# matsengrp/linearham

Measured on AMD Instinct MI355X. Metric: phylo-HMM log-likelihood evals/sec (100-leaf x 400-site family), higher is better.
Workload: dtype f64

## Files before the change

### linearham_amd/csrc/lh_prune.hip

```cpp
#include <cstdlib>

#include <cstdio>

#include "lh_device.h"

namespace lh {

namespace {

thread_local char g_prune_form[64] = "";
thread_local char g_prune_error[256] = "";

#define LH_SLOT_COPY(dst, src)                       \
  _Pragma("unroll") for (int s_ = 0; s_ < S; ++s_) { \
    dst[s_][0] = src[s_][0];                         \
    dst[s_][1] = src[s_][1];                         \
    dst[s_][2] = src[s_][2];                         \
    dst[s_][3] = src[s_][3];                         \
  }
#define LH_PUSH_IF(d)                                   \
  if constexpr (kDepth > d) {                           \
    if (push_mask & (1u << d)) { LH_SLOT_COPY(st##d, a) } \
  }
#define LH_POP_CASE(d)          \
  case d:                       \
    if constexpr (kDepth > d) { \
      LH_SLOT_COPY(y, st##d)    \
    }                           \
    break;
#define LH_POP_SLOT(d) \
  _Pragma("unroll") for (int s_ = 0; s_ < S; ++s_) matvec(pa, st##d[s_], z[s_]);
#define LH_DECL(d) double st##d[S][4];

typedef const double __attribute__((address_space(4))) * pmat_ptr;


__device__ __forceinline__ pmat_ptr pmat_after_barrier(const double* p) {
  const uint64_t bits = reinterpret_cast<uint64_t>(p);
  const uint32_t lo = (uint32_t)__builtin_amdgcn_readfirstlane((int)(uint32_t)bits);
  const uint32_t hi = (uint32_t)__builtin_amdgcn_readfirstlane((int)(uint32_t)(bits >> 32));
  uint64_t v = (uint64_t)lo | ((uint64_t)hi << 32);
  asm volatile("; lh: P-matrix scratch base %0 -- scalar loads of the walk depend on this statement" : "+s"(v) : : "memory");
  return (pmat_ptr)v;
}

__device__ __forceinline__ void matvec(pmat_ptr p, const double (&a)[4], double (&x)[4]) {
  x[0] = fma(p[3], a[3], fma(p[2], a[2], fma(p[1], a[1], p[0] * a[0])));
  x[1] = fma(p[7], a[3], fma(p[6], a[2], fma(p[5], a[1], p[4] * a[0])));
  x[2] = fma(p[11], a[3], fma(p[10], a[2], fma(p[9], a[1], p[8] * a[0])));
  x[3] = fma(p[15], a[3], fma(p[14], a[2], fma(p[13], a[1], p[12] * a[0])));
}

template <bool kN>
__device__ __forceinline__ void tip_column(const double* tiptab, int tip, int st, double (&c)[4], int ones_off) {
  const int off = tip * 16 + st * 4;
// ... 199 lines not shown
  const double2 q0 = q[0], q1 = q[1];
  c[0] = q0.x, c[1] = q0.y, c[2] = q1.x, c[3] = q1.y;
}

typedef int2 WalkOp;
enum : int { WOP_MATRIX = 8, WOP_PUSH_SHIFT = 4, WOP_POP_SHIFT = 9, WOP_HAS_B = 1 << 13, WOP_HAS_C = 1 << 14 };


template <bool kN>
__device__ __forceinline__ void tip_column_at(const char* tiptab_bytes, int entry_off, int st, double (&c)[4], int ones_off) {
  const int off = entry_off + st * 32;
  const double2* q = reinterpret_cast<const double2*>(tiptab_bytes + ((kN && st == 4) ? ones_off * 8 : off));
  const double2 q0 = q[0], q1 = q[1];
  c[0] = q0.x, c[1] = q0.y, c[2] = q1.x, c[3] = q1.y;
}

template <bool kN>
__device__ __forceinline__ void table_entry_at(const char* ctab_bytes, unsigned table_off, int sy, int sz, double (&c)[4]) {
  constexpr int SY = kN ? 5 : 4;
  const unsigned off = table_off + (unsigned)(sy * SY + sz) * 32u;
  const double2* q = reinterpret_cast<const double2*>(ctab_bytes + off);
  const double2 q0 = q[0], q1 = q[1];
  c[0] = q0.x, c[1] = q0.y, c[2] = q1.x, c[3] = q1.y;
}

template <int S>
__device__ __forceinline__ void close_naive_branch(const double (&a)[S][4], const int (&scal)[S], const double* naive_tab,
                                                   const double* __restrict__ p4, double (&lik)[S][5], int (&scl)[S]) {
#pragma unroll
  for (int s = 0; s < S; ++s) {
    const double w0 = p4[0] * a[s][0], w1 = p4[1] * a[s][1], w2 = p4[2] * a[s][2], w3 = p4[3] * a[s][3];
#pragma unroll
    for (int b = 0; b < 5; ++b) {
      double tv[4];
      if (b < 4) {
#pragma unroll
        for (int i = 0; i < 4; ++i) tv[i] = naive_tab[b * 4 + i];
      } else {
#pragma unroll
        for (int i = 0; i < 4; ++i) tv[i] = ((naive_tab[i] + naive_tab[4 + i]) + naive_tab[8 + i]) + naive_tab[12 + i];
      }
      lik[s][b] = fma(w3, tv[3], fma(w2, tv[2], fma(w1, tv[1], w0 * tv[0])));
    }
    scl[s] = scal[s];
  }
}

typedef __attribute__((address_space(5))) char* private_ptr;
typedef __attribute__((address_space(3))) const char* lds_ptr;

template <int kDepth, bool kN, int S>
__device__ __forceinline__ void prune_wave_asm(int block128, const uint64_t* __restrict__ planes, int n_blocks, int n_w,
                                               const WalkOp* __restrict__ wops, pmat_ptr pm, unsigned ctoff,
                                               const double* tiptab, const double* naive_tab, const double* ones,
                                               const double* __restrict__ p4, double (&lik)[S][5], int (&scl)[S]) {
  static_assert(S == 1 || S == 2, "one or two sites per lane");
  __attribute__((aligned(16))) double out_mem[4 * S + 2];
  __attribute__((aligned(16))) double deep_mem[(kDepth > 2 ? kDepth - 2 : 1) * 4 * S];
  constexpr int kMasks = kN ? 6 : 4;
  const int blk = min(block128, n_blocks - 1);
  const uint64_t* planes_w = planes + ((ptrdiff_t)blk - (ptrdiff_t)n_blocks) * kMasks;
  const unsigned pstride = (unsigned)n_blocks * (unsigned)(kMasks * 8);
  const unsigned tip_lds = (unsigned)(size_t)(lds_ptr)tiptab;
  if constexpr (kN && S == 2) {
    const unsigned ones_lds = (unsigned)(size_t)(lds_ptr)ones;
    asm volatile(
#include "lh_prune_walk_asm_s2n.inc"
        :
        : [nw] "s"(n_w), [wops] "s"(wops), [pm] "s"(pm), [ctoff] "s"(ctoff), [planes] "s"(planes_w), [pstride] "s"(pstride),
          [tip] "s"(tip_lds), [ones] "v"(ones_lds), [out] "v"((private_ptr)out_mem), [deep] "v"((private_ptr)deep_mem)
        : "memory", "vcc", "scc",
#include "lh_prune_walk_clobbers_s2.inc"
    );
  } else if constexpr (S == 2) {
    asm volatile(
#include "lh_prune_walk_asm_s2.inc"
        :
        : [nw] "s"(n_w), [wops] "s"(wops), [pm] "s"(pm), [ctoff] "s"(ctoff), [planes] "s"(planes_w), [pstride] "s"(pstride),
          [tip] "s"(tip_lds), [out] "v"((private_ptr)out_mem), [deep] "v"((private_ptr)deep_mem)
        : "memory", "vcc", "scc",
#include "lh_prune_walk_clobbers_s2.inc"
    );
  } else if constexpr (kN) {
    const unsigned ones_lds = (unsigned)(size_t)(lds_ptr)ones;
    asm volatile(
#include "lh_prune_walk_asm_s1n.inc"
        :
        : [nw] "s"(n_w), [wops] "s"(wops), [pm] "s"(pm), [ctoff] "s"(ctoff), [planes] "s"(planes_w), [pstride] "s"(pstride),
          [tip] "s"(tip_lds), [ones] "v"(ones_lds), [out] "v"((private_ptr)out_mem), [deep] "v"((private_ptr)deep_mem)
        : "memory", "vcc", "scc",
#include "lh_prune_walk_clobbers_s1.inc"
    );
  } else {
    asm volatile(
#include "lh_prune_walk_asm_s1.inc"
        :
        : [nw] "s"(n_w), [wops] "s"(wops), [pm] "s"(pm), [ctoff] "s"(ctoff), [planes] "s"(planes_w), [pstride] "s"(pstride),
          [tip] "s"(tip_lds), [out] "v"((private_ptr)out_mem), [deep] "v"((private_ptr)deep_mem)
        : "memory", "vcc", "scc",
#include "lh_prune_walk_clobbers_s1.inc"
    );
  }
  double a[S][4];
  int scal[S];
#pragma unroll
  for (int s = 0; s < S; ++s)
#pragma unroll
    for (int i = 0; i < 4; ++i) a[s][i] = out_mem[s * 4 + i];
  const unsigned* packed = reinterpret_cast<const unsigned*>(out_mem + 4 * S);
#pragma unroll
  for (int s = 0; s < S; ++s) scal[s] = (int)((packed[s / 2] >> (16 * (s & 1))) & 0xffffu);
  close_naive_branch<S>(a, scal, naive_tab, p4, lik, scl);
}

template <int kDepth, int S, bool kN>
__device__ __forceinline__ void prune_wave_ct(int site0, int site_end, const uint8_t* __restrict__ msa, int L, int n_w,
                                              const WalkOp* desc , pmat_ptr pm, const double* tiptab,
                                              const double* ctab, const double* naive_tab, int ones_off,
                                              const double* __restrict__ p4, double (&lik)[S][5], int (&scl)[S]) {
  constexpr unsigned kTabBytes = (kN ? 25 : 16) * 32;
  unsigned usite[S];
#pragma unroll
  for (int s = 0; s < S; ++s) {
    const int site = site0 + 64 * s;
    usite[s] = (unsigned)(site < site_end ? site : site_end - 1);
  }
  double a[S][4];
  int scal[S];
#pragma unroll
  for (int s = 0; s < S; ++s) {
    a[s][0] = a[s][1] = a[s][2] = a[s][3] = 1.0;
    scal[s] = 0;
  }
  double st0[S][4];
  double deep[kDepth > 1 ? kDepth - 1 : 1][S][4];
#pragma unroll
  for (int s = 0; s < S; ++s) st0[s][0] = st0[s][1] = st0[s][2] = st0[s][3] = 0.0;
  const char* tipb = reinterpret_cast<const char*>(tiptab);
  const char* ctabb = reinterpret_cast<const char*>(ctab);
  const uint8_t* msa_m = msa - L;
  const int last = n_w > 0 ? n_w - 1 : 0;
  WalkOp d0, d1, dv;
  {
    const WalkOp t0 = desc[0], t1 = desc[last < 1 ? last : 1];
    d0.x = __builtin_amdgcn_readfirstlane(t0.x), d0.y = __builtin_amdgcn_readfirstlane(t0.y);
    d1.x = __builtin_amdgcn_readfirstlane(t1.x), d1.y = __builtin_amdgcn_readfirstlane(t1.y);
    dv = desc[last < 2 ? last : 2];
  }
  int sa[S], sb[S], sc[S];
#pragma unroll
  for (int s = 0; s < S; ++s) sa[s] = sb[s] = sc[s] = 0;
  if (n_w > 0) {
#pragma unroll
    for (int s = 0; s < S; ++s) {
      sa[s] = msa_m[(unsigned)(((unsigned)d0.x >> 16) * L) + usite[s]];
      sb[s] = msa_m[(unsigned)((d0.y & 0xffff) * L) + usite[s]];
      sc[s] = msa_m[(unsigned)(((unsigned)d0.y >> 16) * L) + usite[s]];
    }
  }
  unsigned pm_off = 0, tab_off = 0;
  for (int k = 0; k < n_w; ++k) {
    const int kind = d0.x & 7;
    const int tip_a = (unsigned)d0.x >> 16, tip_b = d0.y & 0xffff, tip_c = (unsigned)d0.y >> 16;
    double x[S][4];
    if (d0.x & WOP_MATRIX) {
// ... 438 lines not shown
      atomicOr(err_flag, 1);
    } else {
      hdr[smp] = make_int4(c_wi, c_mi, c_ti, 0);
    }
  }
  if (any_bad) return;
  __syncthreads();
  for (int c = lane; c < c_ti; c += 64) ml[c_mi + c] = bl[tnode[c]];
}

__global__ void __launch_bounds__(64) schedule_stack_check_kernel(int T, int slots, int check_ranks,
                                                                  const int32_t* __restrict__ ops, int4* __restrict__ hdr,
                                                                  int32_t* err_flag) {
  const int smp = blockIdx.x, lane = threadIdx.x;
  const int n_ops = T - 2, nodes = 2 * T - 2;
  const int4* __restrict__ o = reinterpret_cast<const int4*>(ops) + (size_t)smp * n_ops;
  int carry = 0, depth0 = 0;
  bool bad = false;
  for (int k0 = 0; k0 < n_ops; k0 += 64) {
    const int k = k0 + lane;
    const bool in = k < n_ops;
    const int4 op = in ? o[k] : make_int4(OP_CHERRY, 1, 1, 0);
    const int kind = op.x & 15, rank = op.x >> OP_RANK_SHIFT;
    const bool push = (op.x & OP_PUSH_FLAG) != 0;
    bool ok = op.x >= 0 && (op.x & 0xe0) == 0 && kind <= OP_POP_ACC;
    if (kind == OP_CHERRY) ok = ok && op.y >= 1 && op.y < T && op.z >= 1 && op.z < T && push == (k != 0);
    if (kind == OP_TIP_ACC) ok = ok && !push && k > 0 && op.y >= 1 && op.y < T && op.z >= T && op.z < nodes;
    if (kind == OP_POP_ACC) ok = ok && !push && k > 0 && op.y >= T && op.y < nodes && op.z >= T && op.z < nodes;
    if (push || kind == OP_POP_ACC) ok = ok && op.w >= 0 && op.w < slots;
    const int m = !in || !ok ? 0 : kind == OP_TIP_ACC ? 1 : kind == OP_POP_ACC ? 2 : 0;
    const int dl = !in || !ok ? 0 : push ? 1 : kind == OP_POP_ACC ? -1 : 0;
    int incl = m, dincl = dl;
#pragma unroll
    for (int d = 1; d < 64; d <<= 1) {
      const int up = __shfl_up(incl, d), dup = __shfl_up(dincl, d);
      if (lane >= d) incl += up, dincl += dup;
    }
    const int depth = depth0 + dincl - dl;
    if (in && push && op.w != depth) ok = false;
    if (in && kind == OP_POP_ACC && op.w != depth - 1) ok = false;
    if (check_ranks && in && kind != OP_CHERRY && rank != carry + incl - m) ok = false;
    if (in && !ok) bad = true;
    carry += __shfl(incl, 63);
    depth0 += __shfl(dincl, 63);
  }
  if (carry != T - 3 || depth0 != 0) bad = true;
  const bool any_bad = __builtin_amdgcn_ballot_w64(bad) != 0;
  if (lane == 0) {
    hdr[smp] = make_int4(0, 0, 0, any_bad ? 1 : 0);
    if (any_bad) atomicOr(err_flag, 1);
  }
}

template <int kDepth, bool kN, bool kFused, bool kAsm = false>
__device__ __forceinline__ void prune_body_ct(int n2, int tile, int R, int wpr, const uint8_t* __restrict__ msa,
                                              const uint64_t* __restrict__ planes, int L,
                                              int T, const int2* __restrict__ wops, const double* __restrict__ wlen,
                                              const int4* __restrict__ tabs, int tabs_stride,
                                              const int4* __restrict__ hdr, const double* __restrict__ brlen,
                                              const double* __restrict__ rates, const double* __restrict__ eig,
                                              double* pmat_w, size_t rate_stride, const double* __restrict__ pi,
                                              double* __restrict__ site_lik, int32_t* __restrict__ site_scal) {
  extern __shared__ double2 smem2[];
  constexpr int SY = kN ? 5 : 4, E = SY * SY;
  const int tid = threadIdx.x;
  const int wave_all = __builtin_amdgcn_readfirstlane(tid >> 6);
  const int rate = kFused ? wave_all / wpr : (int)blockIdx.y;
  const int wave = kFused ? wave_all - rate * wpr : wave_all;
  const int nthr = kFused ? wpr * 64 : (int)blockDim.x;
  const int rtid = kFused ? tid - rate * nthr : tid;
  const int sample = blockIdx.z;
  const int n_ops = T - 2;
  const int4 h = hdr[sample];
  const int n_w = __builtin_amdgcn_readfirstlane(h.x);
  const int n_mat = __builtin_amdgcn_readfirstlane(h.y), n_tab = __builtin_amdgcn_readfirstlane(h.z);
  const bool malformed = h.w != 0;
  double* pw = pmat_w + ((size_t)sample * R + rate) * rate_stride;
  double* ctab = pw + (size_t)(T - 3 > 0 ? T - 3 : 0) * 16;
  constexpr int kS = 2;
  double* tiptab = reinterpret_cast<double*>(smem2) + (kFused ? (size_t)rate * T * 16 : 0);
  const double* naive_tab = tiptab;
  double* ones = reinterpret_cast<double*>(smem2) + (size_t)(kFused ? R : 1) * T * 16;
  const int ones_off = (int)(ones - tiptab);
  if (kN && tid < 4) ones[tid] = 1.0;
  const int4* __restrict__ tl = tabs + (size_t)sample * tabs_stride;
  WalkOp* desc = reinterpret_cast<WalkOp*>(reinterpret_cast<double*>(smem2) + (size_t)(kFused ? R : 1) * T * 16 + (kN ? 4 : 0));
  for (int i = tid; i < n_w; i += blockDim.x) desc[i] = wops[(size_t)sample * n_ops + i];

  const int n_q = min(n_tab, nthr >> 2);
  const bool pc_lane = (rtid & 3) == 0 && (rtid >> 2) < n_q;
  int4 tcell = make_int4(1, 1, 0, 0);
  if ((rtid >> 2) < n_q) tcell = tl[rtid >> 2];
  double pcq[16];
#pragma unroll
  for (int i = 0; i < 16; ++i) pcq[i] = 0.0;
  {
    const double* __restrict__ e = eig + (size_t)sample * 36;
    const double* __restrict__ bl = brlen + (size_t)sample * (2 * (size_t)T - 2);
    const double* __restrict__ wl = wlen + (size_t)sample * n_ops;
    const int n_rest = n_tab - n_q;
    const int n_list = n_mat + n_rest + T;
    const int round1 = nthr - n_q;
    auto item = [&](bool is_pc, int it, int rr, int quad) {
      double P[4][4];
      const bool in_list = !is_pc && it < n_list;
      const bool inner = in_list && it < n_mat + n_rest;
      const int slot = it < n_mat ? it : it + n_q;
      const int j = it - (n_mat + n_rest);
      double t = 0.0;
      if (is_pc) t = wl[n_mat + quad];
      else if (inner) t = wl[slot];
      else if (in_list) t = bl[j];
      compute_pmatrix(e, t * rates[(size_t)sample * R + rr], P);
      if (is_pc) {
#pragma unroll
        for (int i = 0; i < 4; ++i)
#pragma unroll
          for (int q = 0; q < 4; ++q) pcq[i * 4 + q] = P[i][q];
      } else if (inner) {
        double* o = pmat_w + ((size_t)sample * R + rr) * rate_stride + (size_t)slot * 16;
#pragma unroll
        for (int i = 0; i < 4; ++i)
#pragma unroll
          for (int q = 0; q < 4; ++q) o[i * 4 + q] = P[i][q];
      } else if (in_list) {
        double* o = reinterpret_cast<double*>(smem2) + (kFused ? (size_t)rr * T * 16 : 0) + j * 16;
#pragma unroll
        for (int i = 0; i < 4; ++i)
#pragma unroll
          for (int st = 0; st < 4; ++st) o[st * 4 + i] = P[i][st];
      }
    };
    const int rem = n_list - round1;
    if (rem > 0) {
      if constexpr (kFused) {
        const float inv_rem = 1.0f / (float)rem;
        for (int c = tid; c < R * rem; c += blockDim.x) {
          int rr = min((int)(((float)c + 0.5f) * inv_rem), R - 1);
          rr -= rr * rem > c ? 1 : 0;
          rr += (rr + 1) * rem <= c ? 1 : 0;
          item(false, round1 + c - rr * rem, rr, 0);
        }
      } else {
        for (int it = round1 + rtid; it < n_list; it += nthr) item(false, it, rate, 0);
      }
    }
    item(pc_lane, rtid - min(n_q, (rtid + 3) >> 2), rate, rtid >> 2);
  }
  if (n_tab > n_q) asm volatile("s_waitcnt vmcnt(0)" ::: "memory");
  asm volatile("s_waitcnt lgkmcnt(0)\n\ts_barrier" ::: "memory");
  auto build_rows = [&](const double (&pc)[16], int c, int sy, int ty, int tz) {
    double py[4];
    tip_column<kN>(tiptab, ty, sy, py, ones_off);
    double2* o = reinterpret_cast<double2*>(ctab) + ((size_t)c * E + (size_t)sy * SY) * 2;
#pragma unroll
    for (int sz = 0; sz < SY; ++sz) {
      double pz[4], pr[4], x[4];
      tip_column<kN>(tiptab, tz, sz, pz, ones_off);
#pragma unroll
      for (int i = 0; i < 4; ++i) pr[i] = py[i] * pz[i];
      matvec_v(pc, pr, x);
      o[2 * sz] = make_double2(x[0], x[1]);
      o[2 * sz + 1] = make_double2(x[2], x[3]);
    }
  };
  {
    double pc[16];
#pragma unroll
    for (int i = 0; i < 16; ++i) {
      const int lo = __builtin_amdgcn_mov_dpp(__double2loint(pcq[i]), 0, 0xf, 0xf, true);
      const int hi = __builtin_amdgcn_mov_dpp(__double2hiint(pcq[i]), 0, 0xf, 0xf, true);
      pc[i] = __hiloint2double(hi, lo);
    }
    if ((rtid >> 2) < n_q) {
      build_rows(pc, rtid >> 2, rtid & 3, tcell.x, tcell.y);
      if constexpr (kN) {
        const int sz = rtid & 3;
        double2* o = reinterpret_cast<double2*>(ctab) + ((size_t)(rtid >> 2) * E + 4 * SY) * 2;
        for (int k = sz; k < SY; k += 4) {
          double pz[4], pr[4], x[4];
          tip_column<kN>(tiptab, tcell.y, k, pz, ones_off);
#pragma unroll
          for (int i = 0; i < 4; ++i) pr[i] = 1.0 * pz[i];
          matvec_v(pc, pr, x);
          o[2 * k] = make_double2(x[0], x[1]);
          o[2 * k + 1] = make_double2(x[2], x[3]);
        }
      }
    }
  }
  for (int it = rtid; it < (n_tab - n_q) * SY; it += nthr) {
    const int c = n_q + it / SY, sy = it - (it / SY) * SY;
    const int4 t = tl[c];
    double pc[16];
    const double2* q = reinterpret_cast<const double2*>(pw + (size_t)(n_mat + c) * 16);
#pragma unroll
    for (int j = 0; j < 8; ++j) {
      const double2 v = q[j];
      pc[2 * j] = v.x;
      pc[2 * j + 1] = v.y;
    }
    build_rows(pc, c, sy, t.x, t.y);
  }
  asm volatile("s_waitcnt vmcnt(0)" ::: "memory");
  __threadfence_block();
  __syncthreads();

  const pmat_ptr pm = pmat_after_barrier(pw);
  const int lane = tid & 63;
  const int tile0 = blockIdx.x * tile;
  const int site_end = min(tile0 + tile, L);
  const double* __restrict__ p4 = pi + (size_t)sample * 4;
  double lik[kS][5];
  int scl[kS];
#pragma unroll
  for (int s = 0; s < kS; ++s) scl[s] = 0;
  int site0, n_own;
  const bool two_sites = wave < n2;
  if (two_sites) {
    site0 = tile0 + wave * (64 * kS) + lane;
    n_own = kS;
    if constexpr (kAsm)
      prune_wave_asm<kDepth, kN, kS>((tile0 + wave * (64 * kS)) >> 7, planes, (L + 127) >> 7, n_w, wops + (size_t)sample * n_ops, pm,
                                     (unsigned)((T - 3 > 0 ? T - 3 : 0) * 128), tiptab, naive_tab, ones, p4, lik, scl);
    else
      prune_wave_ct<kDepth, kS, kN>(site0, site_end, msa, L, n_w, desc, pm, tiptab, ctab, naive_tab, ones_off, p4, lik, scl);
  } else {
    site0 = tile0 + n2 * (64 * kS) + (wave - n2) * 64 + lane;
    n_own = 1;
    double lik1[1][5];
    int scl1[1];
    if constexpr (kAsm)
      prune_wave_asm<kDepth, kN, 1>((tile0 + n2 * (64 * kS)) >> 7, planes, (L + 127) >> 7, n_w,
                                    wops + (size_t)sample * n_ops, pm, (unsigned)((T - 3 > 0 ? T - 3 : 0) * 128), tiptab, naive_tab,
                                    ones, p4, lik1, scl1);
    else
      prune_wave_ct<kDepth, 1, kN>(site0, site_end, msa, L, n_w, desc, pm, tiptab, ctab, naive_tab, ones_off, p4, lik1, scl1);
#pragma unroll
    for (int b = 0; b < 5; ++b) lik[0][b] = lik1[0][b];
    scl[0] = scl1[0];
  }
  if (malformed) {
#pragma unroll
    for (int s = 0; s < kS; ++s)
#pragma unroll
      for (int b = 0; b < 5; ++b) lik[s][b] = __builtin_nan("");
  }

  if constexpr (!kFused) {
    double* lik_out = site_lik + (((size_t)sample * R + rate) * 5) * (size_t)L;
    int32_t* scal_out = site_scal + ((size_t)sample * R + rate) * (size_t)L;
#pragma unroll
    for (int s = 0; s < kS; ++s) {
      const int site = site0 + 64 * s;
      if (s < n_own && site < site_end) {
#pragma unroll
        for (int b = 0; b < 5; ++b) lik_out[(size_t)b * L + site] = lik[s][b];
        scal_out[site] = scl[s];
      }
    }
  } else {
    const int pad = n2 * (64 * kS) + (wpr - n2) * 64;
    __syncthreads();
    double* X = reinterpret_cast<double*>(smem2);
    int* SC = reinterpret_cast<int*>(X + (size_t)R * 5 * pad);
#pragma unroll
    for (int s = 0; s < kS; ++s) {
      const int idx = site0 + 64 * s - tile0;
      if (s < n_own && idx < pad) {
#pragma unroll
        for (int b = 0; b < 5; ++b) X[((size_t)rate * 5 + b) * pad + idx] = lik[s][b];
        SC[rate * pad + idx] = scl[s];
      }
    }
    __syncthreads();
    const int n_tile = site_end - tile0;
    const double w = 1.0 / R;
    double* lik_out = site_lik + ((size_t)sample * 5) * (size_t)L;
    int32_t* scal_out = site_scal + (size_t)sample * (size_t)L;
    for (int p = tid; p < n_tile; p += blockDim.x) {
      int smin = 0x7fffffff;
      for (int r = 0; r < R; ++r) smin = min(smin, SC[r * pad + p]);
      double acc[5] = {0.0, 0.0, 0.0, 0.0, 0.0};
      for (int r = 0; r < R; ++r) {
        const int d = SC[r * pad + p] - smin;
#pragma unroll
        for (int b = 0; b < 5; ++b) {
          double v = X[((size_t)r * 5 + b) * pad + p];
          for (int q = 0; q < d && v != 0.0; ++q) v *= kScaleThreshold;
          acc[b] += w * v;
        }
      }
#pragma unroll
      for (int b = 0; b < 5; ++b) lik_out[(size_t)b * L + tile0 + p] = acc[b];
      scal_out[tile0 + p] = smin;
    }
  }
}

#define LH_PRUNE_CT_PARAMS                                                                                          \
  int n2, int tile, int R, int wpr, const uint8_t *__restrict__ msa, const uint64_t *__restrict__ planes, int L,    \
      int T, const int2 *__restrict__ wops,                                                                         \
      const double *__restrict__ wlen, const int4 *__restrict__ tabs, int tabs_stride,                              \
      const int4 *__restrict__ hdr, const double *__restrict__ brlen, const double *__restrict__ rates,            \
      const double *__restrict__ eig, double *pmat_w, size_t rate_stride, const double *__restrict__ pi,           \
      double *__restrict__ site_lik, int32_t *__restrict__ site_scal
#define LH_PRUNE_CT_ARGS \
  n2, tile, R, wpr, msa, planes, L, T, wops, wlen, tabs, tabs_stride, hdr, brlen, rates, eig, pmat_w, rate_stride, pi, site_lik, \
      site_scal
#define LH_PRUNE_CT_KERNEL(NAME, WAVES)                                                              \
  template <int kDepth, bool kN, bool kFused, bool kAsm>                                             \
  __global__ void __launch_bounds__(1024) __attribute__((amdgpu_waves_per_eu(WAVES, WAVES))) NAME(   \
      LH_PRUNE_CT_PARAMS) {                                                                          \
    prune_body_ct<kDepth, kN, kFused, kAsm>(LH_PRUNE_CT_ARGS);                                       \
  }
LH_PRUNE_CT_KERNEL(prune_kernel_ct6, 6)
LH_PRUNE_CT_KERNEL(prune_kernel_ct5, 5)
LH_PRUNE_CT_KERNEL(prune_kernel_ct4, 4)
#undef LH_PRUNE_CT_KERNEL
#define LH_PRUNE_PARAMS                                                                                     \
  int n_samples, int n2, int tile, int R, int wpr, const uint8_t *__restrict__ msa, int L, int T, int n_ops, \
      const int32_t *__restrict__ ops, const int4 *__restrict__ hdr, int32_t *err_flag,                     \
      const double *__restrict__ brlen, const double *__restrict__ rates, const double *__restrict__ eig,  \
      double *pmat_w, size_t rate_stride, const double *__restrict__ pi,                                   \
      double *__restrict__ site_lik, int32_t *__restrict__ site_scal
#define LH_PRUNE_ARGS \
  n2, tile, R, wpr, msa, L, T, n_ops, ops, hdr, err_flag, brlen, rates, eig, pmat_w, rate_stride, pi, site_lik, site_scal
#define LH_PRUNE_SAMPLES(BODY) BODY((int)blockIdx.z, LH_PRUNE_ARGS);

#define LH_PRUNE_KERNEL(NAME, WAVES)                                                                 \
  template <int kDepth, bool kN>                                                                     \
  __global__ void __launch_bounds__(1024) __attribute__((amdgpu_waves_per_eu(WAVES, WAVES))) NAME(   \
      LH_PRUNE_PARAMS) {                                                                             \
    LH_PRUNE_SAMPLES((prune_body<kDepth, true, kN, true>))                                           \
  }
LH_PRUNE_KERNEL(prune_kernel_w6, 6)
LH_PRUNE_KERNEL(prune_kernel_w5, 5)
LH_PRUNE_KERNEL(prune_kernel_w4, 4)
#undef LH_PRUNE_KERNEL

template <int kDepth, bool kN>
__global__ void __launch_bounds__(512) __attribute__((amdgpu_waves_per_eu(5, 5))) prune_kernel_seg(LH_PRUNE_PARAMS) {
  LH_PRUNE_SAMPLES((prune_body<kDepth, true, kN, false, true>))
}
template <int kDepth, bool kN>
__global__ void __launch_bounds__(512) __attribute__((amdgpu_waves_per_eu(4, 4))) prune_kernel_seg4(LH_PRUNE_PARAMS) {
  LH_PRUNE_SAMPLES((prune_body<kDepth, true, kN, false, true>))
}

PruneWsSizes prune_ws_sizes(int T, bool mixed_n) {
  PruneWsSizes z;
  z.tabs_per_sample = (size_t)std::max((T - 1) / 2, 1);
  const size_t e = mixed_n ? 25 : 16;
  z.scratch_doubles_per_rate = std::max((size_t)std::max(T - 3, 0) * 16 + z.tabs_per_sample * e * 4, (size_t)std::max(T - 2, 1) * 32);
  return z;
}

int launch_prune(const DevFamily& fam, int n, int R, int T, int max_depth, const int32_t* ops,
                 const double* brlen, const double* rates, const double* eig, const PruneWs& ws, const double* pi,
                 double* site_lik, int32_t* site_scal, hipStream_t stream, bool allow_fused) {
  const int L = fam.n_prune;
  const PruneWsSizes sizes = prune_ws_sizes(T, fam.msa_mixed_n != 0);
  if (L == 0) {
    hipLaunchKernelGGL(schedule_stack_check_kernel, dim3(n), dim3(64), 0, stream, T, std::max(max_depth, 1), 0, ops, ws.hdr, ws.err_flag);
    return R;
  }
  double* pmat = ws.scratch;
  const size_t rate_stride = sizes.scratch_doubles_per_rate;
  const DebugOptions& dbg = debug_options();
  const int cap_env = dbg.k1_tile_cap;
  const int cap = cap_env >= 64 ? std::min(cap_env, 1024) : 1024;
  const int tiles = (L + cap - 1) / cap;
  const int tile = tiles == 1 ? L : (((L + tiles - 1) / tiles + 127) & ~127);
  int n2 = tile / 128, n1;
  {
    const int rem = tile - 128 * n2;
    if (rem > 64) {
      ++n2;
      n1 = 0;
    } else {
      n1 = rem > 0 ? 1 : 0;
    }
  }
  const int wpr = n2 + n1;
  const size_t tip_bytes = (size_t)T * 16 * sizeof(double);
  const size_t pad = (size_t)n2 * 128 + (size_t)n1 * 64;
  const size_t tail_bytes = (((size_t)std::max(T - 2, 1) * sizeof(int2)) + 31) & ~(size_t)15;
  const bool mixed = fam.msa_mixed_n != 0;
  const size_t ones_bytes = mixed ? 32 : 0;
  const size_t fused_lds = std::max((size_t)R * tip_bytes + ones_bytes + tail_bytes, (size_t)R * pad * (5 * sizeof(double) + sizeof(int)));
  const bool fused = allow_fused && !dbg.k1_no_fuse && !dbg.k1_segments &&
                     ((R * wpr <= 8 && fused_lds <= 53 * 1024) ||
                      (R * wpr > 8 && R * wpr <= 16 && fused_lds <= 80 * 1024));
  const bool big = !fused && ((160 * 1024 / tip_bytes) * wpr / 4 < 5 || dbg.k1_segments);
  const bool tables_hook = dbg.k1_tables || dbg.k1_no_tables;
  const bool use_asm = !dbg.k1_cxx_walk;
  const bool stack_fused = fused && max_depth <= 4 && dbg.k1_stack && !tables_hook;
  const bool seg = big && max_depth <= 4 && !tables_hook;
  const size_t seg_bytes = (size_t)(2 * kSegOps + 1) * 16 * sizeof(double) + ones_bytes;
  size_t lds = fused ? fused_lds : seg ? seg_bytes : tip_bytes + ones_bytes + tail_bytes;
  if (lds > 160 * 1024) {
    snprintf(g_prune_error, sizeof(g_prune_error),
             "K1: a tree of %d tips with stack depth %d needs %zu bytes of LDS in the cherry-table form (160 KB per CU)", T, max_depth, lds);
    return -1;
  }
  if (stack_fused || seg) {
    hipLaunchKernelGGL(schedule_stack_check_kernel, dim3(n), dim3(64), 0, stream, T, stack_fused && max_depth <= 3 ? 3 : 4,
                       stack_fused ? 1 : 0, ops, ws.hdr, ws.err_flag);
  } else {
    hipLaunchKernelGGL(schedule_rewrite_kernel, dim3(n), dim3(64), (sizes.tabs_per_sample + 16) * sizeof(int), stream, T, max_depth,
                       (int)sizes.tabs_per_sample, dbg.k1_no_tables ? 0 : 1, ops, brlen, ws.wops, ws.wlen, ws.tabs, ws.hdr, ws.err_flag);
  }
  const int wg_waves = fused ? R * wpr : wpr;
  dim3 grid(tiles, fused ? 1 : R, n), block(64 * wg_waves);
  const int n_ops = T - 2;
  hipError_t attr_rc = hipSuccess;
#define LH_LAUNCH_K(K, NAME)                                                                                     \
  {                                                                                                              \
    if (lds > 64 * 1024)                                                                                         \
      attr_rc = hipFuncSetAttribute(reinterpret_cast<const void*>(K), hipFuncAttributeMaxDynamicSharedMemorySize, (int)lds); \
    snprintf(g_prune_form, sizeof(g_prune_form), "%s", NAME);                                                    \
    if (attr_rc == hipSuccess)                                                                                   \
      hipLaunchKernelGGL(K, grid, block, lds, stream, n, n2, tile, R, wpr, fam.msa, L, T, n_ops, ops, ws.hdr, ws.err_flag, \
                         brlen, rates, eig, pmat, rate_stride, pi, site_lik, site_scal);                        \
  }
#define LH_LAUNCH_CT(K, NAME)                                                                                    \
  {                                                                                                              \
    if (lds > 64 * 1024)                                                                                         \
      attr_rc = hipFuncSetAttribute(reinterpret_cast<const void*>(K), hipFuncAttributeMaxDynamicSharedMemorySize, (int)lds); \
    snprintf(g_prune_form, sizeof(g_prune_form), "%s", NAME);                                                    \
    if (attr_rc == hipSuccess)                                                                                   \
      hipLaunchKernelGGL(K, grid, block, lds, stream, n2, tile, R, wpr, fam.msa, fam.msa_planes, L, T, ws.wops, ws.wlen, ws.tabs, \
                         (int)sizes.tabs_per_sample, ws.hdr, brlen, rates, eig, pmat, rate_stride, pi, site_lik, \
                         site_scal);                                                                             \
  }
  const int lds_waves = lds == 0 ? 8 : (int)((160 * 1024 / lds) * wg_waves / 4);
  if (stack_fused) {
#define LH_LAUNCH_STACK(D, N)                                                          \
  {                                                                                    \
    if (lds_waves >= 6 && D == 3)                                                      \
      LH_LAUNCH_K((prune_kernel_w6<D, N>), "w6<" #D "," #N ">")                        \
    else if (lds_waves >= 5)                                                           \
      LH_LAUNCH_K((prune_kernel_w5<D, N>), "w5<" #D "," #N ">")                        \
    else                                                                               \
      LH_LAUNCH_K((prune_kernel_w4<D, N>), "w4<" #D "," #N ">")                        \
  }
    if (max_depth <= 3 && !mixed)
      LH_LAUNCH_STACK(3, false)
    else if (max_depth <= 3)
      LH_LAUNCH_STACK(3, true)
    else if (!mixed)
      LH_LAUNCH_STACK(4, false)
    else
      LH_LAUNCH_STACK(4, true)
#undef LH_LAUNCH_STACK
  } else if (seg) {
    if (dbg.k1_seg_waves == 4) {
      if (mixed)
        LH_LAUNCH_K((prune_kernel_seg4<4, true>), "seg4<4,true>")
      else
        LH_LAUNCH_K((prune_kernel_seg4<4, false>), "seg4<4,false>")
    } else {
      if (mixed)
        LH_LAUNCH_K((prune_kernel_seg<4, true>), "seg5<4,true>")
      else
        LH_LAUNCH_K((prune_kernel_seg<4, false>), "seg5<4,false>")
    }
  } else {
#define LH_LAUNCH_BUDGET(D, N, F, A)                                                          \
  {                                                                                           \
    if (lds_waves >= 6)                                                                       \
      LH_LAUNCH_CT((prune_kernel_ct6<D, N, F, A>), "ct6<" #D "," #N "," #F "," #A ">")        \
    else if (lds_waves >= 5)                                                                  \
      LH_LAUNCH_CT((prune_kernel_ct5<D, N, F, A>), "ct5<" #D "," #N "," #F "," #A ">")        \
    else                                                                                      \
      LH_LAUNCH_CT((prune_kernel_ct4<D, N, F, A>), "ct4<" #D "," #N "," #F "," #A ">")        \
  }
#define LH_LAUNCH_FORM(D, N, A)        \
  {                                    \
    if (fused)                         \
      LH_LAUNCH_BUDGET(D, N, true, A)  \
    else                               \
      LH_LAUNCH_BUDGET(D, N, false, A) \
  }
#define LH_LAUNCH_SHALLOW(D)           \
  {                                    \
    if (mixed && use_asm)              \
      LH_LAUNCH_FORM(D, true, true)    \
// ... 30 lines not shown
```

Before: 8.107 million.

## Re-read kernel arguments from kernarg segment to cut SGPR/VGPR pressure in prune_body_ct

Packs the prune kernel's many parameters into a struct and has the body reload fields from the kernarg segment (through opaque asm barriers) per phase instead of keeping them live across the asm walk. The naive-branch closing is moved out of the asm wave routine so the walk's register footprint shrinks. It also replaces the integer divide for the fused rate index with a loop or rcp-based estimate and rolls the table-building loop for the non-quad path. The aim is lower register pressure and fewer live values across the barrier, traded for extra scalar loads and some added complexity and risk.

```diff
diff --git a/linearham_amd/csrc/lh_prune.hip b/linearham_amd/csrc/lh_prune.hip
--- a/linearham_amd/csrc/lh_prune.hip
+++ b/linearham_amd/csrc/lh_prune.hip
@@ -1,6 +1,7 @@
 #include <cstdlib>
 
 #include <cstdio>
+#include <type_traits>
 
 #include "lh_device.h"
 
@@ -306,8 +307,7 @@
 template <int kDepth, bool kN, int S>
 __device__ __forceinline__ void prune_wave_asm(int block128, const uint64_t* __restrict__ planes, int n_blocks, int n_w,
                                                const WalkOp* __restrict__ wops, pmat_ptr pm, unsigned ctoff,
-                                               const double* tiptab, const double* naive_tab, const double* ones,
-                                               const double* __restrict__ p4, double (&lik)[S][5], int (&scl)[S]) {
+                                               const double* tiptab, const double* ones, double (&a)[S][4], int (&scal)[S]) {
   static_assert(S == 1 || S == 2, "one or two sites per lane");
   __attribute__((aligned(16))) double out_mem[4 * S + 2];
   __attribute__((aligned(16))) double deep_mem[(kDepth > 2 ? kDepth - 2 : 1) * 4 * S];
@@ -355,8 +355,6 @@
 #include "lh_prune_walk_clobbers_s1.inc"
     );
   }
-  double a[S][4];
-  int scal[S];
 #pragma unroll
   for (int s = 0; s < S; ++s)
 #pragma unroll
@@ -364,7 +362,6 @@
   const unsigned* packed = reinterpret_cast<const unsigned*>(out_mem + 4 * S);
 #pragma unroll
   for (int s = 0; s < S; ++s) scal[s] = (int)((packed[s / 2] >> (16 * (s & 1))) & 0xffffu);
-  close_naive_branch<S>(a, scal, naive_tab, p4, lik, scl);
 }
 
 template <int kDepth, int S, bool kN>
@@ -909,79 +906,123 @@
   }
 }
 
+struct PruneCtArgs {
+  int n2, tile, R, wpr;
+  int L, T, tabs_stride, pad_;
+  const uint8_t* msa;
+  const uint64_t* planes;
+  const int2* wops;
+  const double* wlen;
+  const int4* tabs;
+  const int4* hdr;
+  const double* brlen;
+  const double* rates;
+  const double* eig;
+  double* pmat_w;
+  size_t rate_stride;
+  const double* pi;
+  double* site_lik;
+  int32_t* site_scal;
+};
+typedef const PruneCtArgs __attribute__((address_space(4)))* ct_args_ptr;
+typedef int __attribute__((ext_vector_type(4))) ct_int4;
+
+__device__ __forceinline__ ct_args_ptr ct_args_again(ct_args_ptr p) {
+  uint64_t v = reinterpret_cast<uint64_t>(p);
+  asm volatile("; lh: kernel arguments at %0, read again from here" : "+s"(v));
+  return (ct_args_ptr)v;
+}
+__device__ __forceinline__ ct_args_ptr ct_args() { return ct_args_again((ct_args_ptr)__builtin_amdgcn_kernarg_segment_ptr()); }
+
+template <class T, class U>
+__device__ __forceinline__ const T __attribute__((address_space(4)))* ct_ro(const U* p) {
+  return (const T __attribute__((address_space(4)))*)reinterpret_cast<uint64_t>(p);
+}
+
+struct CtWave {
+  int rate, wave, nthr, rtid;
+};
+constexpr int kCtFusedMaxWaves = 16;
+constexpr size_t kCtFusedMaxLds = 80 * 1024;
+static_assert(kCtFusedMaxWaves <= 16, "ct_wave counts at most 15 steps");
+static_assert(53 * 1024 <= kCtFusedMaxLds, "the limit of fused workgroups of up to eight waves (launch_prune) lies within it");
+static_assert(3 * (kCtFusedMaxLds / 128) < (1u << 21), "prune_body_ct: c / rem through v_rcp_f32 needs R * rem < 2^21");
+template <bool kFused>
+__device__ __forceinline__ int ct_block_threads(int R, int wpr) {
+  return (kFused ? R : 1) * wpr * 64;
+}
+template <bool kFused>
+__device__ __forceinline__ CtWave ct_wave(int tid, int wpr) {
+  const int wave_all = __builtin_amdgcn_readfirstlane(tid >> 6);
+  if constexpr (kFused) {
+    int rate = 0, wave = wave_all;
+    for (; wave >= wpr && rate < 15; ++rate) wave -= wpr;
+    return CtWave{rate, wave, wpr * 64, tid - rate * wpr * 64};
+  } else {
+    return CtWave{(int)blockIdx.y, wave_all, wpr * 64, tid};
+  }
+}
+
 template <int kDepth, bool kN, bool kFused, bool kAsm = false>
-__device__ __forceinline__ void prune_body_ct(int n2, int tile, int R, int wpr, const uint8_t* __restrict__ msa,
-                                              const uint64_t* __restrict__ planes, int L,
-                                              int T, const int2* __restrict__ wops, const double* __restrict__ wlen,
-                                              const int4* __restrict__ tabs, int tabs_stride,
-                                              const int4* __restrict__ hdr, const double* __restrict__ brlen,
-                                              const double* __restrict__ rates, const double* __restrict__ eig,
-                                              double* pmat_w, size_t rate_stride, const double* __restrict__ pi,
-                                              double* __restrict__ site_lik, int32_t* __restrict__ site_scal) {
+__device__ __forceinline__ void prune_body_ct() {
   extern __shared__ double2 smem2[];
   constexpr int SY = kN ? 5 : 4, E = SY * SY;
+  constexpr int kS = 2;
   const int tid = threadIdx.x;
-  const int wave_all = __builtin_amdgcn_readfirstlane(tid >> 6);
-  const int rate = kFused ? wave_all / wpr : (int)blockIdx.y;
-  const int wave = kFused ? wave_all - rate * wpr : wave_all;
-  const int nthr = kFused ? wpr * 64 : (int)blockDim.x;
-  const int rtid = kFused ? tid - rate * nthr : tid;
   const int sample = blockIdx.z;
-  const int n_ops = T - 2;
-  const int4 h = hdr[sample];
-  const int n_w = __builtin_amdgcn_readfirstlane(h.x);
-  const int n_mat = __builtin_amdgcn_readfirstlane(h.y), n_tab = __builtin_amdgcn_readfirstlane(h.z);
-  const bool malformed = h.w != 0;
-  double* pw = pmat_w + ((size_t)sample * R + rate) * rate_stride;
-  double* ctab = pw + (size_t)(T - 3 > 0 ? T - 3 : 0) * 16;
-  constexpr int kS = 2;
-  double* tiptab = reinterpret_cast<double*>(smem2) + (kFused ? (size_t)rate * T * 16 : 0);
-  const double* naive_tab = tiptab;
-  double* ones = reinterpret_cast<double*>(smem2) + (size_t)(kFused ? R : 1) * T * 16;
-  const int ones_off = (int)(ones - tiptab);
-  if (kN && tid < 4) ones[tid] = 1.0;
-  const int4* __restrict__ tl = tabs + (size_t)sample * tabs_stride;
-  WalkOp* desc = reinterpret_cast<WalkOp*>(reinterpret_cast<double*>(smem2) + (size_t)(kFused ? R : 1) * T * 16 + (kN ? 4 : 0));
-  for (int i = tid; i < n_w; i += blockDim.x) desc[i] = wops[(size_t)sample * n_ops + i];
-
-  const int n_q = min(n_tab, nthr >> 2);
-  const bool pc_lane = (rtid & 3) == 0 && (rtid >> 2) < n_q;
+  const ct_args_ptr a0 = ct_args();
+  const CtWave g = ct_wave<kFused>(tid, a0->wpr);
+  const int rate = g.rate, wave = g.wave, nthr = g.nthr, rtid = g.rtid;
+  {
+    const ct_args_ptr a = a0;
+    const int T = a->T, R = a->R;
+    const int n_w = ct_ro<int>(a->hdr)[(size_t)sample * 4];
+    if (kN && tid < 4) reinterpret_cast<double*>(smem2)[(kFused ? R : 1) * T * 16 + tid] = 1.0;
+    const WalkOp* wops = a->wops + (size_t)sample * (T - 2);
+    WalkOp* desc = reinterpret_cast<WalkOp*>(reinterpret_cast<double*>(smem2) + (size_t)(kFused ? R : 1) * T * 16 + (kN ? 4 : 0));
+    for (int i = tid; i < n_w; i += ct_block_threads<kFused>(R, a->wpr))
+      desc[i] = *reinterpret_cast<const WalkOp*>(reinterpret_cast<const char*>(wops) + (unsigned)i * 8u);
+  }
+
   int4 tcell = make_int4(1, 1, 0, 0);
-  if ((rtid >> 2) < n_q) tcell = tl[rtid >> 2];
   double pcq[16];
-#pragma unroll
-  for (int i = 0; i < 16; ++i) pcq[i] = 0.0;
   {
-    const double* __restrict__ e = eig + (size_t)sample * 36;
-    const double* __restrict__ bl = brlen + (size_t)sample * (2 * (size_t)T - 2);
-    const double* __restrict__ wl = wlen + (size_t)sample * n_ops;
+    const ct_args_ptr a = a0;
+    const int T = a->T, R = a->R, n_ops = T - 2;
+    const int n_mat = ct_ro<int>(a->hdr)[(size_t)sample * 4 + 1], n_tab = ct_ro<int>(a->hdr)[(size_t)sample * 4 + 2];
+    const size_t rate_stride = a->rate_stride;
+    const int n_q = min(n_tab, nthr >> 2);
+    const bool in_quad = (rtid >> 2) < n_q;
+    const bool pc_lane = (rtid & 3) == 0 && in_quad;
+    if (in_quad) tcell = (a->tabs + (size_t)sample * a->tabs_stride)[rtid >> 2];
+    const double* bl = a->brlen + (size_t)sample * (2 * (size_t)T - 2);
+    const double* wl = a->wlen + (size_t)sample * n_ops;
+    char* pw_s = reinterpret_cast<char*>(a->pmat_w + (size_t)sample * R * rate_stride);
+    const unsigned rate_bytes = (unsigned)rate_stride * 8u;
     const int n_rest = n_tab - n_q;
-    const int n_list = n_mat + n_rest + T;
+    const int n_in = n_mat + n_rest;
+    const int n_list = n_in + T;
     const int round1 = nthr - n_q;
-    auto item = [&](bool is_pc, int it, int rr, int quad) {
-      double P[4][4];
-      const bool in_list = !is_pc && it < n_list;
-      const bool inner = in_list && it < n_mat + n_rest;
+    auto item = [&](bool listed, bool is_pc, int it, int rr, int quad, double (&P)[4][4]) {
+      const bool in_list = listed || (!is_pc && it < n_list);
+      const bool inner = in_list && it < n_in;
       const int slot = it < n_mat ? it : it + n_q;
-      const int j = it - (n_mat + n_rest);
+      const int j = it - n_in;
       double t = 0.0;
-      if (is_pc) t = wl[n_mat + quad];
-      else if (inner) t = wl[slot];
+      if (is_pc || inner) t = wl[is_pc ? n_mat + quad : slot];
       else if (in_list) t = bl[j];
-      compute_pmatrix(e, t * rates[(size_t)sample * R + rr], P);
-      if (is_pc) {
-#pragma unroll
-        for (int i = 0; i < 4; ++i)
-#pragma unroll
-          for (int q = 0; q < 4; ++q) pcq[i * 4 + q] = P[i][q];
-      } else if (inner) {
-        double* o = pmat_w + ((size_t)sample * R + rr) * rate_stride + (size_t)slot * 16;
+      uint64_t ev = reinterpret_cast<uint64_t>(a->eig + (size_t)sample * 36);
+      asm volatile("; lh: eigen-system at %0" : "+s"(ev));
+      const double* e = (const double*)(const double __attribute__((address_space(4)))*)ev;
+      compute_pmatrix(e, t * ct_ro<double>(a->rates)[(size_t)sample * R + rr], P);
+      if (inner) {
+        double* o = reinterpret_cast<double*>(pw_s + ((unsigned)rr * rate_bytes + (unsigned)slot * 128u));
 #pragma unroll
         for (int i = 0; i < 4; ++i)
 #pragma unroll
           for (int q = 0; q < 4; ++q) o[i * 4 + q] = P[i][q];
       } else if (in_list) {
-        double* o = reinterpret_cast<double*>(smem2) + (kFused ? (size_t)rr * T * 16 : 0) + j * 16;
+        double* o = reinterpret_cast<double*>(smem2) + (kFused ? rr * T * 16 : 0) + j * 16;
 #pragma unroll
         for (int i = 0; i < 4; ++i)
 #pragma unroll
@@ -990,27 +1031,49 @@
     };
     const int rem = n_list - round1;
     if (rem > 0) {
+      double P[4][4];
       if constexpr (kFused) {
-        const float inv_rem = 1.0f / (float)rem;
-        for (int c = tid; c < R * rem; c += blockDim.x) {
-          int rr = min((int)(((float)c + 0.5f) * inv_rem), R - 1);
-          rr -= rr * rem > c ? 1 : 0;
-          rr += (rr + 1) * rem <= c ? 1 : 0;
-          item(false, round1 + c - rr * rem, rr, 0);
+        const float inv_rem = __builtin_amdgcn_rcpf((float)rem);
+        for (int c = tid; c < R * rem; c += ct_block_threads<kFused>(R, a->wpr)) {
+          const int rr = (int)(((float)c + 0.5f) * inv_rem);
+          item(true, false, round1 + c - rr * rem, rr, 0, P);
         }
       } else {
-        for (int it = round1 + rtid; it < n_list; it += nthr) item(false, it, rate, 0);
-      }
-    }
-    item(pc_lane, rtid - min(n_q, (rtid + 3) >> 2), rate, rtid >> 2);
-  }
-  if (n_tab > n_q) asm volatile("s_waitcnt vmcnt(0)" ::: "memory");
+        for (int it = round1 + rtid; it < n_list; it += nthr) item(true, false, it, rate, 0, P);
+      }
+    }
+    double P[4][4];
+    item(false, pc_lane, rtid - min(n_q, (rtid + 3) >> 2), rate, rtid >> 2, P);
+#pragma unroll
+    for (int i = 0; i < 4; ++i)
+#pragma unroll
+      for (int q = 0; q < 4; ++q) pcq[i * 4 + q] = P[i][q];
+    if (n_tab > n_q) asm volatile("s_waitcnt vmcnt(0)" ::: "memory");
+  }
   asm volatile("s_waitcnt lgkmcnt(0)\n\ts_barrier" ::: "memory");
-  auto build_rows = [&](const double (&pc)[16], int c, int sy, int ty, int tz) {
+  const ct_args_ptr a = ct_args_again(a0);
+  int tid2 = tid;
+  asm volatile("" : "+v"(tid2));
+  const int rtid2 = kFused ? tid2 - rate * nthr : tid2;
+  const int T = a->T, R = a->R;
+  const int n_w = ct_ro<int>(a->hdr)[(size_t)sample * 4];
+  const int n_mat = ct_ro<int>(a->hdr)[(size_t)sample * 4 + 1], n_tab = ct_ro<int>(a->hdr)[(size_t)sample * 4 + 2];
+  const int n_q = min(n_tab, nthr >> 2);
+  const bool in_quad = (rtid2 >> 2) < n_q;
+  double* pw = a->pmat_w + ((size_t)sample * R + rate) * a->rate_stride;
+  double* ctab = pw + (size_t)(T - 3 > 0 ? T - 3 : 0) * 16;
+  double* tiptab = reinterpret_cast<double*>(smem2) + (kFused ? (size_t)rate * T * 16 : 0);
+  double* ones = reinterpret_cast<double*>(smem2) + (size_t)(kFused ? R : 1) * T * 16;
+  const int ones_off = (int)(ones - tiptab);
+  const int4* tl = a->tabs + (size_t)sample * a->tabs_stride;
+  const WalkOp* wops = a->wops + (size_t)sample * (T - 2);
+  const WalkOp* desc = reinterpret_cast<const WalkOp*>(ones + (kN ? 4 : 0));
+  auto build_rows = [&](auto rolled, const double (&pc)[16], int c, int sy, int ty, int tz) {
+    constexpr int kUnroll = decltype(rolled)::value ? 1 : SY;
     double py[4];
     tip_column<kN>(tiptab, ty, sy, py, ones_off);
-    double2* o = reinterpret_cast<double2*>(ctab) + ((size_t)c * E + (size_t)sy * SY) * 2;
-#pragma unroll
+    double2* o = reinterpret_cast<double2*>(reinterpret_cast<char*>(ctab) + ((unsigned)c * E + (unsigned)sy * SY) * 32u);
+#pragma unroll kUnroll
     for (int sz = 0; sz < SY; ++sz) {
       double pz[4], pr[4], x[4];
       tip_column<kN>(tiptab, tz, sz, pz, ones_off);
@@ -1021,7 +1084,7 @@
       o[2 * sz + 1] = make_double2(x[2], x[3]);
     }
   };
-  {
+  if (wave * 16 < n_q) {
     double pc[16];
 #pragma unroll
     for (int i = 0; i < 16; ++i) {
@@ -1029,11 +1092,11 @@
       const int hi = __builtin_amdgcn_mov_dpp(__double2hiint(pcq[i]), 0, 0xf, 0xf, true);
       pc[i] = __hiloint2double(hi, lo);
     }
-    if ((rtid >> 2) < n_q) {
-      build_rows(pc, rtid >> 2, rtid & 3, tcell.x, tcell.y);
+    if (in_quad) {
+      build_rows(std::false_type(), pc, rtid2 >> 2, rtid2 & 3, tcell.x, tcell.y);
       if constexpr (kN) {
-        const int sz = rtid & 3;
-        double2* o = reinterpret_cast<double2*>(ctab) + ((size_t)(rtid >> 2) * E + 4 * SY) * 2;
+        const int sz = rtid2 & 3;
+        double2* o = reinterpret_cast<double2*>(reinterpret_cast<char*>(ctab) + ((unsigned)(rtid2 >> 2) * E + 4 * SY) * 32u);
         for (int k = sz; k < SY; k += 4) {
           double pz[4], pr[4], x[4];
           tip_column<kN>(tiptab, tcell.y, k, pz, ones_off);
@@ -1046,130 +1109,153 @@
       }
     }
   }
-  for (int it = rtid; it < (n_tab - n_q) * SY; it += nthr) {
+  for (int it = rtid2; it < (n_tab - n_q) * SY; it += nthr) {
     const int c = n_q + it / SY, sy = it - (it / SY) * SY;
     const int4 t = tl[c];
     double pc[16];
-    const double2* q = reinterpret_cast<const double2*>(pw + (size_t)(n_mat + c) * 16);
+    const double2* q = reinterpret_cast<const double2*>(reinterpret_cast<const char*>(pw) + (unsigned)(n_mat + c) * 128u);
 #pragma unroll
     for (int j = 0; j < 8; ++j) {
       const double2 v = q[j];
       pc[2 * j] = v.x;
       pc[2 * j + 1] = v.y;
     }
-    build_rows(pc, c, sy, t.x, t.y);
+    build_rows(std::true_type(), pc, c, sy, t.x, t.y);
   }
   asm volatile("s_waitcnt vmcnt(0)" ::: "memory");
   __threadfence_block();
   __syncthreads();
 
-  const pmat_ptr pm = pmat_after_barrier(pw);
-  const int lane = tid & 63;
-  const int tile0 = blockIdx.x * tile;
-  const int site_end = min(tile0 + tile, L);
-  const double* __restrict__ p4 = pi + (size_t)sample * 4;
   double lik[kS][5];
   int scl[kS];
 #pragma unroll
   for (int s = 0; s < kS; ++s) scl[s] = 0;
-  int site0, n_own;
-  const bool two_sites = wave < n2;
-  if (two_sites) {
-    site0 = tile0 + wave * (64 * kS) + lane;
-    n_own = kS;
-    if constexpr (kAsm)
-      prune_wave_asm<kDepth, kN, kS>((tile0 + wave * (64 * kS)) >> 7, planes, (L + 127) >> 7, n_w, wops + (size_t)sample * n_ops, pm,
-                                     (unsigned)((T - 3 > 0 ? T - 3 : 0) * 128), tiptab, naive_tab, ones, p4, lik, scl);
-    else
-      prune_wave_ct<kDepth, kS, kN>(site0, site_end, msa, L, n_w, desc, pm, tiptab, ctab, naive_tab, ones_off, p4, lik, scl);
-  } else {
-    site0 = tile0 + n2 * (64 * kS) + (wave - n2) * 64 + lane;
-    n_own = 1;
-    double lik1[1][5];
-    int scl1[1];
-    if constexpr (kAsm)
-      prune_wave_asm<kDepth, kN, 1>((tile0 + n2 * (64 * kS)) >> 7, planes, (L + 127) >> 7, n_w,
-                                    wops + (size_t)sample * n_ops, pm, (unsigned)((T - 3 > 0 ? T - 3 : 0) * 128), tiptab, naive_tab,
-                                    ones, p4, lik1, scl1);
-    else
-      prune_wave_ct<kDepth, 1, kN>(site0, site_end, msa, L, n_w, desc, pm, tiptab, ctab, naive_tab, ones_off, p4, lik1, scl1);
-#pragma unroll
-    for (int b = 0; b < 5; ++b) lik[0][b] = lik1[0][b];
-    scl[0] = scl1[0];
-  }
-  if (malformed) {
+  double root[kS][4];
+  int root_scal[kS];
+  int tid_w = tid2;
+  if constexpr (kAsm) asm volatile("v_mov_b32 %0, %1" : "=v"(tid_w) : "v"(tid2));
+  {
+    const pmat_ptr pm = pmat_after_barrier(pw);
+    const int L = a->L, n2 = a->n2;
+    const int tile0 = blockIdx.x * a->tile;
+    if (wave < n2) {
+      if constexpr (kAsm)
+        prune_wave_asm<kDepth, kN, kS>((tile0 + wave * (64 * kS)) >> 7, a->planes, (L + 127) >> 7, n_w, wops, pm,
+                                       (unsigned)((T - 3 > 0 ? T - 3 : 0) * 128), tiptab, ones, root, root_scal);
+      else
+        prune_wave_ct<kDepth, kS, kN>(tile0 + wave * (64 * kS) + (tid2 & 63), min(tile0 + a->tile, L), a->msa, L, n_w, desc, pm,
+                                      tiptab, ctab, tiptab, ones_off, (const double*)(ct_ro<double>(a->pi) + (size_t)sample * 4), lik, scl);
+    } else {
+      double lik1[1][5], root1[1][4];
+      int scl1[1], root_scal1[1];
+      if constexpr (kAsm) {
+        prune_wave_asm<kDepth, kN, 1>((tile0 + n2 * (64 * kS)) >> 7, a->planes, (L + 127) >> 7, n_w, wops, pm,
+                                      (unsigned)((T - 3 > 0 ? T - 3 : 0) * 128), tiptab, ones, root1, root_scal1);
+#pragma unroll
+        for (int i = 0; i < 4; ++i) root[0][i] = root1[0][i];
+        root_scal[0] = root_scal1[0];
+      } else {
+        prune_wave_ct<kDepth, 1, kN>(tile0 + n2 * (64 * kS) + (wave - n2) * 64 + (tid2 & 63), min(tile0 + a->tile, L), a->msa, L, n_w,
+                                     desc, pm, tiptab, ctab, tiptab, ones_off, (const double*)(ct_ro<double>(a->pi) + (size_t)sample * 4), lik1, scl1);
+#pragma unroll
+        for (int b = 0; b < 5; ++b) lik[0][b] = lik1[0][b];
+        scl[0] = scl1[0];
+      }
+    }
+  }
+
+  const ct_args_ptr b = ct_args_again(a);
+  int tid_b = tid_w;
+  if constexpr (kAsm) asm volatile("v_mov_b32 %0, %1" : "=v"(tid_b) : "v"(tid_w));
+  const CtWave gb = ct_wave<kFused>(tid_b, b->wpr);
+  const int rate_b = gb.rate, wave_b = gb.wave;
+  const int R_b = b->R, L_b = b->L, n2_b = b->n2;
+  const int lane = tid_b & 63;
+  const int tile0 = blockIdx.x * b->tile;
+  const int site_end = min(tile0 + b->tile, L_b);
+  const bool two_sites = wave_b < n2_b;
+  const int site0 = two_sites ? tile0 + wave_b * (64 * kS) + lane : tile0 + n2_b * (64 * kS) + (wave_b - n2_b) * 64 + lane;
+  const int n_own = two_sites ? kS : 1;
+  if constexpr (kAsm) {
+    const double* naive_tab = reinterpret_cast<const double*>(smem2) + (kFused ? (size_t)rate_b * b->T * 16 : 0);
+    const double* p4 = (const double*)(ct_ro<double>(b->pi) + (size_t)sample * 4);
+    if (two_sites) {
+      close_naive_branch<kS>(root, root_scal, naive_tab, p4, lik, scl);
+    } else {
+      double lik1[1][5], root1[1][4];
+      int scl1[1], root_scal1[1];
+#pragma unroll
+      for (int i = 0; i < 4; ++i) root1[0][i] = root[0][i];
+      root_scal1[0] = root_scal[0];
+      close_naive_branch<1>(root1, root_scal1, naive_tab, p4, lik1, scl1);
+#pragma unroll
+      for (int q = 0; q < 5; ++q) lik[0][q] = lik1[0][q];
+      scl[0] = scl1[0];
+    }
+  }
+  if (ct_ro<ct_int4>(b->hdr)[sample].w != 0) {
 #pragma unroll
     for (int s = 0; s < kS; ++s)
 #pragma unroll
-      for (int b = 0; b < 5; ++b) lik[s][b] = __builtin_nan("");
+      for (int q = 0; q < 5; ++q) lik[s][q] = __builtin_nan("");
   }
 
   if constexpr (!kFused) {
-    double* lik_out = site_lik + (((size_t)sample * R + rate) * 5) * (size_t)L;
-    int32_t* scal_out = site_scal + ((size_t)sample * R + rate) * (size_t)L;
+    double* lik_out = b->site_lik + (((size_t)sample * R_b + rate_b) * 5) * (size_t)L_b;
+    int32_t* scal_out = b->site_scal + ((size_t)sample * R_b + rate_b) * (size_t)L_b;
 #pragma unroll
     for (int s = 0; s < kS; ++s) {
       const int site = site0 + 64 * s;
       if (s < n_own && site < site_end) {
 #pragma unroll
-        for (int b = 0; b < 5; ++b) lik_out[(size_t)b * L + site] = lik[s][b];
+        for (int q = 0; q < 5; ++q) lik_out[(size_t)q * L_b + site] = lik[s][q];
         scal_out[site] = scl[s];
       }
     }
   } else {
-    const int pad = n2 * (64 * kS) + (wpr - n2) * 64;
+    const int pad = n2_b * (64 * kS) + (b->wpr - n2_b) * 64;
     __syncthreads();
     double* X = reinterpret_cast<double*>(smem2);
-    int* SC = reinterpret_cast<int*>(X + (size_t)R * 5 * pad);
+    int* SC = reinterpret_cast<int*>(X + (size_t)R_b * 5 * pad);
 #pragma unroll
     for (int s = 0; s < kS; ++s) {
       const int idx = site0 + 64 * s - tile0;
       if (s < n_own && idx < pad) {
 #pragma unroll
-        for (int b = 0; b < 5; ++b) X[((size_t)rate * 5 + b) * pad + idx] = lik[s][b];
-        SC[rate * pad + idx] = scl[s];
+        for (int q = 0; q < 5; ++q) X[((size_t)rate_b * 5 + q) * pad + idx] = lik[s][q];
+        SC[rate_b * pad + idx] = scl[s];
       }
     }
     __syncthreads();
     const int n_tile = site_end - tile0;
-    const double w = 1.0 / R;
-    double* lik_out = site_lik + ((size_t)sample * 5) * (size_t)L;
-    int32_t* scal_out = site_scal + (size_t)sample * (size_t)L;
-    for (int p = tid; p < n_tile; p += blockDim.x) {
+    const double w = 1.0 / R_b;
+    double* lik_out = b->site_lik + ((size_t)sample * 5) * (size_t)L_b;
+    int32_t* scal_out = b->site_scal + (size_t)sample * (size_t)L_b;
+    for (int p = tid_b; p < n_tile; p += ct_block_threads<kFused>(R_b, b->wpr)) {
       int smin = 0x7fffffff;
-      for (int r = 0; r < R; ++r) smin = min(smin, SC[r * pad + p]);
+      for (int r = 0; r < R_b; ++r) smin = min(smin, SC[r * pad + p]);
       double acc[5] = {0.0, 0.0, 0.0, 0.0, 0.0};
-      for (int r = 0; r < R; ++r) {
+      for (int r = 0; r < R_b; ++r) {
         const int d = SC[r * pad + p] - smin;
 #pragma unroll
-        for (int b = 0; b < 5; ++b) {
-          double v = X[((size_t)r * 5 + b) * pad + p];
-          for (int q = 0; q < d && v != 0.0; ++q) v *= kScaleThreshold;
-          acc[b] += w * v;
+        for (int q = 0; q < 5; ++q) {
+          double v = X[((size_t)r * 5 + q) * pad + p];
+          for (int k = 0; k < d && v != 0.0; ++k) v *= kScaleThreshold;
+          acc[q] += w * v;
         }
       }
 #pragma unroll
-      for (int b = 0; b < 5; ++b) lik_out[(size_t)b * L + tile0 + p] = acc[b];
+      for (int q = 0; q < 5; ++q) lik_out[(size_t)q * L_b + tile0 + p] = acc[q];
       scal_out[tile0 + p] = smin;
     }
   }
 }
 
-#define LH_PRUNE_CT_PARAMS                                                                                          \
-  int n2, int tile, int R, int wpr, const uint8_t *__restrict__ msa, const uint64_t *__restrict__ planes, int L,    \
-      int T, const int2 *__restrict__ wops,                                                                         \
-      const double *__restrict__ wlen, const int4 *__restrict__ tabs, int tabs_stride,                              \
-      const int4 *__restrict__ hdr, const double *__restrict__ brlen, const double *__restrict__ rates,            \
-      const double *__restrict__ eig, double *pmat_w, size_t rate_stride, const double *__restrict__ pi,           \
-      double *__restrict__ site_lik, int32_t *__restrict__ site_scal
-#define LH_PRUNE_CT_ARGS \
-  n2, tile, R, wpr, msa, planes, L, T, wops, wlen, tabs, tabs_stride, hdr, brlen, rates, eig, pmat_w, rate_stride, pi, site_lik, \
-      site_scal
 #define LH_PRUNE_CT_KERNEL(NAME, WAVES)                                                              \
   template <int kDepth, bool kN, bool kFused, bool kAsm>                                             \
   __global__ void __launch_bounds__(1024) __attribute__((amdgpu_waves_per_eu(WAVES, WAVES))) NAME(   \
-      LH_PRUNE_CT_PARAMS) {                                                                          \
-    prune_body_ct<kDepth, kN, kFused, kAsm>(LH_PRUNE_CT_ARGS);                                       \
+      const PruneCtArgs args ) {                                         \
+    prune_body_ct<kDepth, kN, kFused, kAsm>();                                                       \
   }
 LH_PRUNE_CT_KERNEL(prune_kernel_ct6, 6)
 LH_PRUNE_CT_KERNEL(prune_kernel_ct5, 5)
@@ -1248,7 +1334,7 @@
   const size_t fused_lds = std::max((size_t)R * tip_bytes + ones_bytes + tail_bytes, (size_t)R * pad * (5 * sizeof(double) + sizeof(int)));
   const bool fused = allow_fused && !dbg.k1_no_fuse && !dbg.k1_segments &&
                      ((R * wpr <= 8 && fused_lds <= 53 * 1024) ||
-                      (R * wpr > 8 && R * wpr <= 16 && fused_lds <= 80 * 1024));
+                      (R * wpr > 8 && R * wpr <= kCtFusedMaxWaves && fused_lds <= kCtFusedMaxLds));
   const bool big = !fused && ((160 * 1024 / tip_bytes) * wpr / 4 < 5 || dbg.k1_segments);
   const bool tables_hook = dbg.k1_tables || dbg.k1_no_tables;
   const bool use_asm = !dbg.k1_cxx_walk;
@@ -1286,11 +1372,16 @@
     if (lds > 64 * 1024)                                                                                         \
       attr_rc = hipFuncSetAttribute(reinterpret_cast<const void*>(K), hipFuncAttributeMaxDynamicSharedMemorySize, (int)lds); \
     snprintf(g_prune_form, sizeof(g_prune_form), "%s", NAME);                                                    \
-    if (attr_rc == hipSuccess)                                                                                   \
-      hipLaunchKernelGGL(K, grid, block, lds, stream, n2, tile, R, wpr, fam.msa, fam.msa_planes, L, T, ws.wops, ws.wlen, ws.tabs, \
-                         (int)sizes.tabs_per_sample, ws.hdr, brlen, rates, eig, pmat, rate_stride, pi, site_lik, \
-                         site_scal);                                                                             \
-  }
+    if (attr_rc == hipSuccess) hipLaunchKernelGGL(K, grid, block, lds, stream, ct_args);                        \
+  }
+  PruneCtArgs ct_args = {};
+  ct_args.n2 = n2, ct_args.tile = tile, ct_args.R = R, ct_args.wpr = wpr;
+  ct_args.L = L, ct_args.T = T, ct_args.tabs_stride = (int)sizes.tabs_per_sample;
+  ct_args.msa = fam.msa, ct_args.planes = fam.msa_planes;
+  ct_args.wops = ws.wops, ct_args.wlen = ws.wlen, ct_args.tabs = ws.tabs, ct_args.hdr = ws.hdr;
+  ct_args.brlen = brlen, ct_args.rates = rates, ct_args.eig = eig;
+  ct_args.pmat_w = pmat, ct_args.rate_stride = rate_stride;
+  ct_args.pi = pi, ct_args.site_lik = site_lik, ct_args.site_scal = site_scal;
   const int lds_waves = lds == 0 ? 8 : (int)((160 * 1024 / lds) * wg_waves / 4);
   if (stack_fused) {
 #define LH_LAUNCH_STACK(D, N)                                                          \
```

Result: faster. 8.251 million (median of 6 runs) (+1.8%).
